# aleju/face-generator

Hardware: AMD Instinct MI355X
Metric: GAN train images/sec (G+D step) at 32x32x3 bs128 (higher is better)
Workload: dtype f32

## Files before the change

### face_generator_amd/csrc/igemm.hip

```cpp
#include "fg_internal.h"
#include <stdio.h>
#include <stdlib.h>

typedef float f32x16 __attribute__((ext_vector_type(16)));

__device__ __forceinline__ void fg_decode_m(int m, int lgH, int lgW, int Hm, int Wm, int& n, int& y, int& x) {
    if (lgW >= 0) {
        x = m & (Wm - 1);
        y = (m >> lgW) & (Hm - 1);
        n = m >> (lgW + lgH);
    } else {
        x = m % Wm;
        int t = m / Wm;
        y = t % Hm;
        n = t / Hm;
    }
}

typedef unsigned int u32x4 __attribute__((ext_vector_type(4)));
#define FG_OOB 0x7FFFFFF0
#define FG_ROW_MASKED 0x20000000

typedef float f32x2 __attribute__((ext_vector_type(2)));
typedef float f32x4 __attribute__((ext_vector_type(4)));
// ... 1720 lines not shown
        }
        for (; s < S; ++s) sum += b[(size_t)s * tile];
    };
    if (wm.kind == 0) {
        run(Part + (size_t)wi * S * tile + e);
    } else {
        for (int p = 0; p < 4; ++p) {
            const int ty = dev_fold_r(p >> 1, dy, wm.pad) - wm.rmin;
            const int tx = dev_fold_r(p & 1, dx, wm.pad) - wm.rmin;
            const int pg = p * wm.G + ty * wm.T + tx;
            run(Part + (size_t)pg * S * tile + e);
        }
    }
    float* gw = gradW + ((size_t)o * wm.I + i) * wm.k * wm.k + wi;
    *gw = (beta == 0.f) ? sum : beta * (*gw) + sum;
}
__host__ __device__ static inline bool fg_finish_all_taps(const WeightMap& wm) { return !wm.wino && wm.kind == 0 && (wm.k == 3 || wm.k == 5); }
__host__ __device__ static inline int fg_finish_taps_tpb(int S) { return S >= 12 ? 32 : 128; }
template <int K>
__device__ __forceinline__ void wgrad_finish_taps(const WeightMap& wm, const float* __restrict__ Part, int S, int Npad, int Cpad,
                                                  float beta, float* __restrict__ gradW, int bx, int po, float* sh) {
    constexpr int kk = K * K;
    const int tpb = fg_finish_taps_tpb(S), ngrp = 128 / tpb;
    const int il = (int)threadIdx.x % tpb, q = (int)threadIdx.x / tpb;
    const int pi = bx * tpb + il;
    const size_t tile = (size_t)Npad * Cpad;
    const int per = (S + ngrp - 1) / ngrp, s0 = q * per, s1 = min(S, s0 + per);
    float sum[kk];
#pragma unroll
    for (int wi = 0; wi < kk; ++wi) sum[wi] = 0.f;
    if (pi < wm.I && po < wm.O) {
        const float* __restrict__ b = Part + (size_t)po * Cpad + pi;
        int s = s0;
        for (; s + 2 <= s1; s += 2) {
            float v0[kk], v1[kk];
#pragma unroll
            for (int wi = 0; wi < kk; ++wi) {
                v0[wi] = b[((size_t)wi * S + s) * tile];
                v1[wi] = b[((size_t)wi * S + s + 1) * tile];
            }
#pragma unroll
            for (int wi = 0; wi < kk; ++wi) { sum[wi] += v0[wi]; sum[wi] += v1[wi]; }
        }
        if (s < s1) {
#pragma unroll
            for (int wi = 0; wi < kk; ++wi) sum[wi] += b[((size_t)wi * S + s) * tile];
        }
    }
#pragma unroll
    for (int wi = 0; wi < kk; ++wi) sh[(q * tpb + il) * kk + wi] = sum[wi];
    __syncthreads();
    if (po >= wm.O) return;
    const int nI = min(tpb, wm.I - bx * tpb);
    float* __restrict__ base = gradW + ((size_t)po * wm.I + (size_t)bx * tpb) * kk;
    for (int idx = (int)threadIdx.x; idx < nI * kk; idx += 128) {
        float t = sh[idx];
        for (int g = 1; g < ngrp; ++g) t += sh[g * tpb * kk + idx];
        base[idx] = (beta == 0.f) ? t : beta * base[idx] + t;
    }
}
__device__ __forceinline__ void wgrad_finish_taps_any(const WeightMap& wm, const float* __restrict__ Part, int S, int Npad, int Cpad,
                                                      float beta, float* __restrict__ gradW, int bx, int po, float* sh) {
    if (wm.k == 5) wgrad_finish_taps<5>(wm, Part, S, Npad, Cpad, beta, gradW, bx, po, sh);
    else wgrad_finish_taps<3>(wm, Part, S, Npad, Cpad, beta, gradW, bx, po, sh);
}
#define FG_WINO_FINISH_LDS (25 * 128)
__host__ __device__ static inline int fg_wino_finish_tpu(const WeightMap& wm) { return (wm.kind == 1 || wm.wino == 2) ? 32 : 128; }
template <int K>
__device__ __forceinline__ void wino_wgrad_finish_block(const WeightMap& wm, const float* __restrict__ Part, int S, int Npad, int Cpad,
                                                        float beta, float* __restrict__ gradW, int bx, int o, float* sh) {
    const int units = (wm.kind == 1 ? 4 : 1) * (wm.wino == 2 ? 4 : 1);
    const int tpu = fg_wino_finish_tpu(wm);
    const int tid = threadIdx.x, u = units == 1 ? 0 : tid / tpu, il = units == 1 ? tid : tid - u * tpu;
    const int i = bx * tpu + il;
    const bool live = i < wm.I && o < wm.O;
    const size_t tile = (size_t)Npad * Cpad;
    float g[K * K];
#pragma unroll
    for (int q = 0; q < K * K; ++q) g[q] = 0.f;
    if (live) {
        float du[16];
#pragma unroll
        for (int pos = 0; pos < 16; ++pos) du[pos] = 0.f;
        const float4* __restrict__ b = (const float4*)(Part + ((size_t)u * S * tile + (size_t)o * Cpad + i) * 16);
        int s = 0;
        for (; s + 4 <= S; s += 4) {
            float4 v[4][4];
#pragma unroll
            for (int e = 0; e < 4; ++e)
#pragma unroll
                for (int q = 0; q < 4; ++q) v[e][q] = b[(size_t)(s + e) * tile * 4 + q];
#pragma unroll
            for (int e = 0; e < 4; ++e)
#pragma unroll
                for (int q = 0; q < 4; ++q) { du[4 * q] += v[e][q].x; du[4 * q + 1] += v[e][q].y; du[4 * q + 2] += v[e][q].z; du[4 * q + 3] += v[e][q].w; }
        }
        for (; s < S; ++s) {
            float4 v[4];
#pragma unroll
            for (int q = 0; q < 4; ++q) v[q] = b[(size_t)s * tile * 4 + q];
#pragma unroll
            for (int q = 0; q < 4; ++q) { du[4 * q] += v[q].x; du[4 * q + 1] += v[q].y; du[4 * q + 2] += v[q].z; du[4 * q + 3] += v[q].w; }
        }
#pragma unroll
        for (int pos = 0; pos < 16; ++pos)
            if (((pos >> 2) == 3) != ((pos & 3) == 3)) du[pos] = -du[pos];
        float r[4][3], t[9];
#pragma unroll
        for (int ii = 0; ii < 4; ++ii) {
            const float d0 = du[ii * 4], d1 = du[ii * 4 + 1], d2 = du[ii * 4 + 2], d3 = du[ii * 4 + 3];
            r[ii][0] = d0 + 0.5f * (d1 + d2);
            r[ii][1] = 0.5f * (d1 - d2);
            r[ii][2] = 0.5f * (d1 + d2) + d3;
        }
#pragma unroll
        for (int bb = 0; bb < 3; ++bb) {
            t[0 * 3 + bb] = r[0][bb] + 0.5f * (r[1][bb] + r[2][bb]);
            t[1 * 3 + bb] = 0.5f * (r[1][bb] - r[2][bb]);
            t[2 * 3 + bb] = 0.5f * (r[1][bb] + r[2][bb]) + r[3][bb];
        }
        if (K == 5 && wm.wino == 2) {
#pragma unroll
            for (int dy = 0; dy < 3; ++dy)
#pragma unroll
                for (int dx = 0; dx < 3; ++dx)
#pragma unroll
                    for (int q = 0; q < K * K; ++q)
                        g[q] = (q == (3 * (u >> 1) + dy) * K + 3 * (u & 1) + dx && 3 * (u >> 1) + dy < K && 3 * (u & 1) + dx < K) ? t[dy * 3 + dx] : g[q];
        } else if (wm.kind == 1) {
#pragma unroll
            for (int dy = 0; dy < K; ++dy)
#pragma unroll
                for (int dx = 0; dx < K; ++dx) {
                    const int ty = dev_fold_r(u >> 1, dy, wm.pad) - wm.rmin, tx = dev_fold_r(u & 1, dx, wm.pad) - wm.rmin;
                    float v = 0.f;
#pragma unroll
                    for (int q = 0; q < 9; ++q) v = (ty * 3 + tx == q) ? t[q] : v;
                    g[dy * K + dx] = v;
                }
        } else if (K == 3) {
#pragma unroll
            for (int q = 0; q < 9; ++q) g[q] = t[q];
        }
    }
    if (units > 1) {
#pragma unroll
        for (int q = 0; q < K * K; ++q) sh[q * 128 + tid] = g[q];
        __syncthreads();
        if (u != 0 || !live) return;
#pragma unroll
        for (int q = 0; q < K * K; ++q) g[q] = ((sh[q * 128 + il] + sh[q * 128 + tpu + il]) + sh[q * 128 + 2 * tpu + il]) + sh[q * 128 + 3 * tpu + il];
    } else if (!live) return;
    float* gw = gradW + ((size_t)o * wm.I + i) * (K * K);
#pragma unroll
    for (int q = 0; q < K * K; ++q) gw[q] = (beta == 0.f) ? g[q] : beta * gw[q] + g[q];
}
__device__ __forceinline__ void wino_wgrad_finish_any(const WeightMap& wm, const float* __restrict__ Part, int S, int Npad, int Cpad,
                                                      float beta, float* __restrict__ gradW, int bx, int o, float* sh) {
    if (wm.k == 5) wino_wgrad_finish_block<5>(wm, Part, S, Npad, Cpad, beta, gradW, bx, o, sh);
    else wino_wgrad_finish_block<3>(wm, Part, S, Npad, Cpad, beta, gradW, bx, o, sh);
}
struct FgWFinishBatch { FgWFinishJob jobs[FG_DEFER_WMAX]; int n; };
__global__ __launch_bounds__(128) void wgrad_finish_jobs_kernel(const FgWFinishBatch b) {
    __shared__ float tl[32][33];
    __shared__ float wsh[FG_WINO_FINISH_LDS];
    int j = 0;
    while (j + 1 < b.n && (long long)blockIdx.x >= b.jobs[j + 1].blk0) ++j;
    const FgWFinishJob& jb = b.jobs[j];
    long long l = (long long)blockIdx.x - jb.blk0;
    if (jb.ib < 0) {
        const WeightMap& wm = jb.wm;
        const int C = wm.i_c, HW = wm.i_hw, nct = (C + 31) / 32, nht = (HW + 31) / 32;
        const int ht = (int)(l % nht); l /= nht;
        const int ct = (int)(l % nct);
        const int po = (int)(l / nct);
        int o = po;
        if (wm.o_hw > 1) { int hw = po / wm.o_c, c = po - hw * wm.o_c; o = c * wm.o_hw + hw; }
        const size_t tile = (size_t)jb.Npad * jb.Cpad;
        const int lx = threadIdx.x & 31, ly = threadIdx.x >> 5;
        for (int r = ly; r < 32; r += 4) {
            const int hw = ht * 32 + r, c = ct * 32 + lx;
            float sum = 0.f;
            if (hw < HW && c < C) {
// ... 489 lines not shown
```

### face_generator_amd/csrc/wino.hip

```cpp
#include "fg_internal.h"
#include <stdio.h>
#include <stdlib.h>
#include <vector>

typedef float f32x16 __attribute__((ext_vector_type(16)));
typedef float f32x4 __attribute__((ext_vector_type(4)));
typedef float f32x2 __attribute__((ext_vector_type(2)));
#define FG_OOB 0x7FFFFFF0

#define WN_STAGE 16384

__device__ __forceinline__ f32x2 wn_load2(__amdgpu_buffer_rsrc_t r, int voff, int soff) {
    return __builtin_bit_cast(f32x2, __builtin_amdgcn_raw_buffer_load_b64(r, voff, soff, 0));
}
__device__ __forceinline__ f32x4 wn_load4(__amdgpu_buffer_rsrc_t r, int voff, int soff) {
    return __builtin_bit_cast(f32x4, __builtin_amdgcn_raw_buffer_load_b128(r, voff, soff, 0));
}
__device__ __forceinline__ f32x2 wn_add(f32x2 a, f32x2 b) {
    f32x2 d;
    asm("v_pk_add_f32 %0, %1, %2" : "=v"(d) : "v"(a), "v"(b));
    return d;
}
__device__ __forceinline__ f32x2 wn_sub(f32x2 a, f32x2 b) {
    f32x2 d;
    asm("v_pk_add_f32 %0, %1, %2 neg_lo:[0,1] neg_hi:[0,1]" : "=v"(d) : "v"(a), "v"(b));
    return d;
}
__device__ __forceinline__ void wn_decode(int t, const WinoArgs& a, int& b, int& ty, int& tx) {
    if (a.lgTW >= 0) {
        tx = t & (a.TW - 1);
        ty = (t >> a.lgTW) & (a.TH - 1);
        b = t >> (a.lgTW + a.lgTH);
    } else {
        tx = t % a.TW;
        const int q = t / a.TW;
        ty = q % a.TH;
        b = q / a.TH;
    }
}

template <int EPI, int TRACE = 0, int DBG = 0>
__device__ __forceinline__ void wino_body(const WinoArgs& a) {
    extern __shared__ __attribute__((aligned(16))) float smem[];
    int* rowoff = (int*)(smem + 2 * WN_STAGE);

    const int tid = threadIdx.x, lane = tid & 63;
    const int wid = __builtin_amdgcn_readfirstlane(tid >> 6);
    const int wm = wid >> 1, wn = wid & 1;
    const int nbn = a.Npad >> 6;
    const int ntn = nbn * a.P;
    const int nmt = (a.T + 63) >> 6;
    int lin = blockIdx.x;
    if ((nmt & 7) == 0) {
        const int xcd = lin & 7, loc = lin >> 3;
        lin = (xcd * (nmt >> 3) + loc / ntn) * ntn + loc % ntn;
    }
    const int tile_m = lin / ntn, cb = lin - tile_m * ntn;
    const int par = cb / nbn, tile_n = cb - par * nbn;
    const int nch = a.C >> 3;
    const int nct = nch * a.KG;
    const int per = (nct + a.splits - 1) / a.splits;
    const int c0 = blockIdx.y * per;
    const int NC = max(0, min(nct, c0 + per) - c0);

    if (tid < 64) {
        const int t = tile_m * 64 + tid;
        int off = -1;
        if (t < a.T) {
            int b, ty, tx;
            wn_decode(t, a, b, ty, tx);
            off = ((b * a.Ho + a.osy * 2 * ty + a.ooy[par]) * a.Wo + a.osx * 2 * tx + a.oox[par]) * a.N;
        }
        rowoff[tid] = off;
    }

    const __amdgpu_buffer_rsrc_t xrsrc = __builtin_amdgcn_make_buffer_rsrc((void*)a.X, 0, (int)a.x_bytes, 0x00020000);
    const __amdgpu_buffer_rsrc_t ursrc = __builtin_amdgcn_make_buffer_rsrc((void*)a.U, 0, FG_OOB, 0x00020000);
    const __amdgpu_buffer_rsrc_t zrsrc = __builtin_amdgcn_make_buffer_rsrc((void*)a.U, 0, 0, 0x00020000);
    const int NCE = (NC + 1) & ~1;
    int voff[16];
    int pb, py0, px0;
    bool tvalid;
    {
        const int t = tile_m * 64 + (tid >> 2);
        int b, ty, tx;
        tvalid = t < a.T;
        wn_decode(tvalid ? t : 0, a, b, ty, tx);
        pb = b * a.Hi; py0 = a.isy * 2 * ty; px0 = a.isx * 2 * tx;
    }
    const int goy4 = *(const int*)a.goy, gox4 = *(const int*)a.gox;
#define WN_GOFF(pk, g) ((int)(signed char)((pk) >> (8 * (g))))
    const int cstep = a.isx * a.C * 4;
#define WN_SET_GROUP(g)                                                                                    \
    {                                                                                                      \
        const int gy_ = py0 + WN_GOFF(goy4, g), gx_ = px0 + WN_GOFF(gox4, g);                              \
        int rb_[4]; bool rok_[4], cok_[4];                                                                 \
        _Pragma("unroll") for (int i = 0; i < 4; ++i) {                                                    \
            const int y = gy_ + a.isy * i;                                                                 \
            rok_[i] = tvalid & ((unsigned)y < (unsigned)a.Hi);                                              \
            rb_[i] = (((pb + y) * a.Wi + gx_) * a.C + 2 * (tid & 3)) * 4;                                  \
            cok_[i] = (unsigned)(gx_ + a.isx * i) < (unsigned)a.Wi;                                        \
        }                                                                                                  \
        _Pragma("unroll") for (int p = 0; p < 16; ++p) voff[p] = (rok_[p >> 2] & cok_[p & 3]) ? rb_[p >> 2] + (p & 3) * cstep : FG_OOB; \
    }
    const int vw = ((tid & 3) >> 1) * 256 + (tid >> 2) * 4 + (tid & 1) * 2;
    const int uo = tid * 4;
    const int ubase = (par * nbn + tile_n) * nct;
    const int a_rd = (lane >> 5) * 256 + (wm * 32 + (lane & 31)) * 4;
    const int b_rd = 8192 + (lane >> 5) * 256 + (wn * 32 + (lane & 31)) * 4;

    int cl = c0, gl = c0 / nch, ccl = c0 - gl * nch;
    WN_SET_GROUP(gl < a.KG ? gl : 0);
#define WN_ADVANCE()                                                                                       \
    {                                                                                                      \
        ++cl;                                                                                              \
        if (++ccl == nch) { ccl = 0; ++gl; if (gl < a.KG) WN_SET_GROUP(gl); }                              \
    }

    f32x2 rva[16], rvb[16];
    f32x4 rua[8], rub[8];
#define WN_LOAD(rv, ru)                                                                                    \
    {                                                                                                      \
        const int sx = ccl * 32, su = (ubase + cl) * 32768;                                                \
        const bool real_ = cl < c0 + NC;                                                                   \
        const __amdgpu_buffer_rsrc_t xr_ = real_ ? xrsrc : zrsrc, ur_ = real_ ? ursrc : zrsrc;             \
        _Pragma("unroll") for (int p = 0; p < 16; ++p) rv[p] = wn_load2(xr_, voff[p], sx);                 \
        _Pragma("unroll") for (int i = 0; i < 8; ++i) ru[i] = wn_load4(ur_, (uo + i * 1024) * 4, su);       \
    }
#define WN_XFORM_STORE(S, rv, ru)                                                                          \
    {                                                                                                      \
        float* Vs = (S) + vw;                                                                              \
        float* Us = (S) + 8192 + uo;                                                                       \
        _Pragma("unroll") for (int i = 0; i < 8; ++i) *(f32x4*)(Us + i * 1024) = ru[i];                    \
        f32x2 w_[16];                                                                                      \
        _Pragma("unroll") for (int x = 0; x < 4; ++x) {                                                    \
            w_[0 + x] = rv[0 + x] - rv[8 + x];                                                             \
            w_[4 + x] = rv[4 + x] + rv[8 + x];                                                             \
            w_[8 + x] = rv[8 + x] - rv[4 + x];                                                             \
            w_[12 + x] = rv[4 + x] - rv[12 + x];                                                           \
        }                                                                                                  \
        _Pragma("unroll") for (int i = 0; i < 4; ++i) {                                                    \
            *(f32x2*)(Vs + (i * 4 + 0) * 512) = w_[i * 4 + 0] - w_[i * 4 + 2];                             \
            *(f32x2*)(Vs + (i * 4 + 1) * 512) = w_[i * 4 + 1] + w_[i * 4 + 2];                             \
            *(f32x2*)(Vs + (i * 4 + 2) * 512) = w_[i * 4 + 2] - w_[i * 4 + 1];                             \
            *(f32x2*)(Vs + (i * 4 + 3) * 512) = w_[i * 4 + 1] - w_[i * 4 + 3];                             \
        }                                                                                                  \
    }

    const int col = tile_n * 64 + wn * 32 + (lane & 31);
    const bool colok = col < a.N;
    const bool bias_late = a.stats_part != nullptr;
    const float bv = (a.bias != nullptr && a.splits == 1 && colok) ? a.bias[col] : 0.f;
    f32x16 acc[16];
#pragma unroll
    for (int p = 0; p < 16; ++p)
#pragma unroll
        for (int r = 0; r < 16; ++r) acc[p][r] = (p == 5 && !bias_late) ? bv : 0.f;

    f32x4 fa[2][2], fb[2][2];
    unsigned long long* trc = nullptr;
    if (TRACE) {
        if (wid == 0 && a.dbg_trace) trc = a.dbg_trace + (size_t)(blockIdx.x + gridDim.x * blockIdx.y) * 128;
        if (trc && lane == 0) trc[0] = __builtin_amdgcn_s_memtime();
    }
    if (NC > 0) {
        WN_LOAD(rva, rua); WN_ADVANCE();
        WN_LOAD(rvb, rub); WN_ADVANCE();
    }
#pragma unroll
    for (int p = 0; p < 16; ++p) asm volatile("" : "+a"(acc[p]));
    __builtin_amdgcn_sched_barrier(0);
    if (NC > 0) {
        WN_XFORM_STORE(smem, rva, rua);
    }
    asm volatile("s_waitcnt lgkmcnt(0)\n\ts_barrier" ::: "memory");
    if (TRACE && trc && lane == 0) trc[1] = __builtin_amdgcn_s_memtime();
    if (NC > 0) {
#pragma unroll
        for (int h = 0; h < 2; ++h) {
            fa[0][h] = *(const f32x4*)(smem + a_rd + h * 512);
            fb[0][h] = *(const f32x4*)(smem + b_rd + h * 512);
        }
    }

#define WN_CHUNK(HAS1, HAS2, RX, UX, RY, UY)                                                               \
    {                                                                                                      \
        const float* Sc = smem + s * WN_STAGE;                                                             \
        float* Sn = smem + (s ^ 1) * WN_STAGE;                                                             \
        float* Vs = Sn + vw;                                                                               \
        float* Us = Sn + 8192 + uo;                                                                        \
        const int sx2 = ccl * 32, su2 = (ubase + cl) * 32768;                                              \
        const bool real_ = cl < c0 + NC;                                                                   \
        const __amdgpu_buffer_rsrc_t xr_ = real_ ? xrsrc : zrsrc, ur_ = real_ ? ursrc : zrsrc;             \
        f32x2 t_;                                                                                          \
        _Pragma("unroll") for (int pr = 0; pr < 8; ++pr) {                                                 \
            _Pragma("unroll") for (int m = 0; m < 8; ++m) {                                                \
                const int sl = pr * 8 + m, h = m & 1, j = m >> 1, pos = 2 * pr + h;                        \
                acc[pos] = __builtin_amdgcn_mfma_f32_32x32x2f32(fa[pr & 1][h][j], fb[pr & 1][h][j], acc[pos], 0, 0, 0); \
                if (TRACE == 2 && (sl & 7) == 0 && ci < 14) {                                              \
                    if (trc && lane == 0) trc[8 + ci * 8 + (sl >> 3)] = __builtin_amdgcn_s_memtime();       \
                }                                                                                          \
                if (m < 4 && pr < 7 && !(DBG & 8)) {                                                       \
                    const int np = 2 * (pr + 1) + (m >> 1);                                                \
                    if ((m & 1) == 0) fa[(pr + 1) & 1][m >> 1] = *(const f32x4*)(Sc + a_rd + np * 512);    \
                    else fb[(pr + 1) & 1][m >> 1] = *(const f32x4*)(Sc + b_rd + np * 512);                 \
                }                                                                                          \
                if (HAS1) {                                                                                \
                    if (m < 4 && pr == 7 && !(DBG & 8)) {                                                  \
                        if ((m & 1) == 0) fa[0][m >> 1] = *(const f32x4*)(Sn + a_rd + (m >> 1) * 512);     \
                        else fb[0][m >> 1] = *(const f32x4*)(Sn + b_rd + (m >> 1) * 512);                  \
                    }                                                                                      \
                    if (sl < 8 && !(DBG & 1)) *(f32x4*)(Us + sl * 1024) = UX[sl];                          \
                    if (HAS2 && !(DBG & 4)) {             \
                        if (sl < 16 && (sl & 1) == 0) UY[sl >> 1] = wn_load4(ur_, (uo + (sl >> 1) * 1024) * 4, su2); \
                        if (sl >= 9 && sl < 41 && (sl & 1) == 1) RY[(sl - 9) >> 1] = wn_load2(xr_, voff[(sl - 9) >> 1], sx2); \
                    }                                                                                      \
                                \
                    if (sl == 8 && !(DBG & 2)) {                                                           \
                        _Pragma("unroll") for (int x = 0; x < 4; ++x) {                                    \
                            RX[0 + x] = wn_sub(RX[0 + x], RX[8 + x]);                                      \
                            RX[12 + x] = wn_sub(RX[4 + x], RX[12 + x]);                                    \
                            t_ = wn_add(RX[4 + x], RX[8 + x]);                                             \
                            RX[8 + x] = wn_sub(RX[8 + x], RX[4 + x]); RX[4 + x] = t_;                      \
                        }                                                                                  \
                    }                                                                                      \
                    if (sl == 10 && !(DBG & 2)) {                                                          \
                        _Pragma("unroll") for (int i = 0; i < 4; ++i) {                                    \
                            RX[i * 4 + 0] = wn_sub(RX[i * 4 + 0], RX[i * 4 + 2]);                          \
                            RX[i * 4 + 3] = wn_sub(RX[i * 4 + 1], RX[i * 4 + 3]);                          \
                            t_ = wn_add(RX[i * 4 + 1], RX[i * 4 + 2]);                                     \
                            RX[i * 4 + 2] = wn_sub(RX[i * 4 + 2], RX[i * 4 + 1]); RX[i * 4 + 1] = t_;      \
                        }                                                                                  \
                    }                                                                                      \
                    if (sl >= 12 && sl < 28 && !(DBG & 2)) *(f32x2*)(Vs + (sl - 12) * 512) = RX[sl - 12];  \
                    if (sl == 55) asm volatile("s_waitcnt lgkmcnt(0)\n\ts_barrier" ::: "memory");          \
                }                                                                                          \
                __builtin_amdgcn_sched_barrier(0);                                                         \
            }                                                                                              \
        }                                                                                                  \
    }
#define WN_STAMP() { if (TRACE == 1 && trc && lane == 0) trc[2 + (ci < 119 ? ci : 119)] = __builtin_amdgcn_s_memtime(); ++ci; }
    int s = 0;
    int ci = 0;
    if (NCE > 0) {
        for (; ci + 2 < NCE;) {
            WN_CHUNK(true, true, rvb, rub, rva, rua); WN_ADVANCE(); WN_STAMP();
            s ^= 1;
            WN_CHUNK(true, true, rva, rua, rvb, rub); WN_ADVANCE(); WN_STAMP();
            s ^= 1;
        }
        WN_CHUNK(true, false, rvb, rub, rva, rua); WN_STAMP();
        s ^= 1;
        WN_CHUNK(false, false, rva, rua, rvb, rub);
        if (ci < NC) WN_STAMP();
    }
#undef WN_STAMP
#undef WN_SET_GROUP
#undef WN_GOFF
#undef WN_ADVANCE
#undef WN_LOAD
#undef WN_XFORM_STORE
#undef WN_CHUNK

    float* outp = a.Out + (size_t)blockIdx.y * a.split_stride;
    const __amdgpu_buffer_rsrc_t orsrc = __builtin_amdgcn_make_buffer_rsrc((void*)outp, 0, FG_OOB, 0x00020000);
    const int oN = a.osx * a.N * 4, oW = a.osy * a.Wo * a.N * 4;
    float sl_ = 0.f, ssum = 0.f, st1 = 0.f, st2 = 0.f;
    if (EPI != 0) sl_ = a.act_slope[0];
    const float badd = bias_late ? bv : 0.f;
#pragma unroll
    for (int r4 = 0; r4 < 4; ++r4) {
        const int4 ro4 = *(const int4*)(rowoff + wm * 32 + 8 * r4 + 4 * (lane >> 5));
        const int ros[4] = {ro4.x, ro4.y, ro4.z, ro4.w};
        float xv[4][4];
        if (EPI == 2) {
            const __amdgpu_buffer_rsrc_t xr = __builtin_amdgcn_make_buffer_rsrc((void*)a.act_x, 0, FG_OOB, 0x00020000);
#pragma unroll
            for (int q = 0; q < 4; ++q) {
                const int vo = (ros[q] >= 0 && colok) ? (ros[q] + col) * 4 : FG_OOB;
                xv[q][0] = __uint_as_float(__builtin_amdgcn_raw_buffer_load_b32(xr, vo, 0, 0));
                xv[q][1] = __uint_as_float(__builtin_amdgcn_raw_buffer_load_b32(xr, vo, oN, 0));
                xv[q][2] = __uint_as_float(__builtin_amdgcn_raw_buffer_load_b32(xr, vo, oW, 0));
                xv[q][3] = __uint_as_float(__builtin_amdgcn_raw_buffer_load_b32(xr, vo, oW + oN, 0));
            }
        }
#pragma unroll
        for (int q = 0; q < 4; ++q) {
            __builtin_amdgcn_sched_barrier(0);
            const int r = r4 * 4 + q;
            float t0[4], t1[4];
#pragma unroll
            for (int j = 0; j < 4; ++j) {
                t0[j] = (acc[0 + j][r] + acc[4 + j][r]) + acc[8 + j][r];
                t1[j] = (acc[4 + j][r] - acc[8 + j][r]) - acc[12 + j][r];
            }
            float y[4];
            y[0] = (t0[0] + t0[1]) + t0[2];
            y[1] = (t0[1] - t0[2]) - t0[3];
            y[2] = (t1[0] + t1[1]) + t1[2];
            y[3] = (t1[1] - t1[2]) - t1[3];
            const int vo = (ros[q] >= 0 && colok) ? (ros[q] + col) * 4 : FG_OOB;
            const int so[4] = {0, oN, oW, oW + oN};
#pragma unroll
            for (int e = 0; e < 4; ++e) {
                if (EPI == 2) {
                    const float x = xv[q][e];
                    const bool pos = x > 0.f;
                    ssum = fmaf(pos ? 0.f : x, y[e], ssum);
                    __builtin_amdgcn_raw_buffer_store_b32(__float_as_uint(pos ? y[e] : sl_ * y[e]), orsrc, vo, so[e], 0);
                } else {
                    if (bias_late) {
                        st1 += y[e];
                        st2 = fmaf(y[e], y[e], st2);
                    }
                    const float yo = y[e] + badd;
                    __builtin_amdgcn_raw_buffer_store_b32(__float_as_uint(yo), orsrc, vo, so[e], 0);
                    if (EPI == 1) {
                        const __amdgpu_buffer_rsrc_t yr = __builtin_amdgcn_make_buffer_rsrc((void*)a.act_y, 0, FG_OOB, 0x00020000);
                        __builtin_amdgcn_raw_buffer_store_b32(__float_as_uint(yo > 0.f ? yo : sl_ * yo), yr, vo, so[e], 0);
                    }
                }
            }
        }
    }
    if (EPI == 2 && a.act_part) {
#pragma unroll
        for (int o = 32; o > 0; o >>= 1) ssum += __shfl_xor(ssum, o, 64);
        if (lane == 0) a.act_part[blockIdx.x * 4 + wid] = ssum;
    }
    if (EPI != 2 && bias_late) {
        st1 += __shfl_xor(st1, 32, 64);
        st2 += __shfl_xor(st2, 32, 64);
        const int row = (tile_m * a.P + par) * 2 + wm;
        if (lane < 32 && colok) {
            a.stats_part[(size_t)row * a.N + col] = st1;
            a.stats_part[((size_t)a.stats_rows + row) * a.N + col] = st2;
        }
    }
    if (TRACE && trc && lane == 0) {
        __builtin_amdgcn_s_waitcnt(0x0f70);
        if (TRACE == 1) trc[(NC < 120 ? NC : 120) + 2] = __builtin_amdgcn_s_memtime();
        trc[127] = (unsigned long long)__builtin_amdgcn_s_getreg(((3 - 1) << 11) | (0 << 6) | 20) | ((unsigned long long)NC << 32);
        trc[126] = (unsigned long long)__builtin_amdgcn_s_getreg(((32 - 1) << 11) | (0 << 6) | 4);
// ... 112 lines not shown
```

### face_generator_amd/csrc/wino_wgrad.hip

```cpp
#include "fg_internal.h"
#include <stdio.h>
#include <stdlib.h>
#include <vector>

typedef float f32x16 __attribute__((ext_vector_type(16)));
typedef float f32x4 __attribute__((ext_vector_type(4)));
typedef float f32x2 __attribute__((ext_vector_type(2)));
#define FG_OOB 0x7FFFFFF0
#define WW_STAGE 16384

__device__ __forceinline__ float ww_load(__amdgpu_buffer_rsrc_t r, int voff, int soff) {
    return __uint_as_float(__builtin_amdgcn_raw_buffer_load_b32(r, voff, soff, 0));
}
__device__ __forceinline__ f32x2 ww_add(f32x2 a, f32x2 b) {
    f32x2 d;
    asm("v_pk_add_f32 %0, %1, %2" : "=v"(d) : "v"(a), "v"(b));
    return d;
}
__device__ __forceinline__ f32x2 ww_sub(f32x2 a, f32x2 b) {
    f32x2 d;
    asm("v_pk_add_f32 %0, %1, %2 neg_lo:[0,1] neg_hi:[0,1]" : "=v"(d) : "v"(a), "v"(b));
    return d;
}

template <int TRACE>
__device__ __forceinline__ void ww_body(const WinoWgradArgs& a) {
    extern __shared__ __attribute__((aligned(16))) float smem[];
    const int tid = threadIdx.x, lane = tid & 63;
    const int wid = __builtin_amdgcn_readfirstlane(tid >> 6);
    const int wm = wid >> 1, wn = wid & 1;
    const int nbc = a.Cpad >> 6;
    const int tn = blockIdx.x / nbc, tc = blockIdx.x - tn * nbc;
    const int pg = blockIdx.z, par = pg / a.KG, grp = pg - par * a.KG;
    const int nct = (a.T + 7) >> 3;
    const int c0 = blockIdx.y * a.chunks_per_split;
    const int NC = max(0, min(nct, c0 + a.chunks_per_split) - c0);
    const int NCE = (NC + 1) & ~1;
    if (NC <= 0) return;
    unsigned long long* trc = nullptr;
    if (TRACE) {
        if (wid == 0 && a.dbg_trace) trc = a.dbg_trace + ((size_t)blockIdx.x + (size_t)gridDim.x * (blockIdx.y + (size_t)gridDim.y * blockIdx.z)) * 128;
        if (trc && lane == 0) trc[0] = __builtin_amdgcn_s_memtime();
    }
    int ci = 0;

    const int dRow = a.osy * a.Wo * a.Nd * 4, dCol = a.osx * a.Nd * 4;
    const int xRow = a.isy * a.Wi * a.Cx * 4, xCol = a.isx * a.Cx * 4;
    const int xShift = 2 * a.Cx * 4;
    const __amdgpu_buffer_rsrc_t drsrc = __builtin_amdgcn_make_buffer_rsrc((void*)a.dY, 0, (int)a.d_bytes, 0x00020000);
    const __amdgpu_buffer_rsrc_t xrsrc = __builtin_amdgcn_make_buffer_rsrc((void*)((const char*)a.X - xShift), 0, (int)a.x_bytes + xShift, 0x00020000);
    const int chD = tn * 64 + lane, chX = tc * 64 + lane;
    const int vD = chD < a.Nd ? chD * 4 : FG_OOB, vX = chX < a.Cx ? chX * 4 : FG_OOB;
    const int goy = a.goy[grp], gox = a.gox[grp], ooy = a.ooy[par], oox = a.oox[par];
    const int cend = c0 + NC;

    const int sw = (wid >> 1) * 256 + lane * 4 + (wid & 1) * 2;
    const int a_rd = (lane >> 5) * 256 + (wm * 32 + (lane & 31)) * 4;
    const int b_rd = 8192 + (lane >> 5) * 256 + (wn * 32 + (lane & 31)) * 4;

    int cl = c0;
    int vrow[4], vdr[2], vo[24], colmask = 0;
    int cur_b = 0, cur_y0 = 0, cur_x0 = 0, cur_dy = 0, cur_dx = 0, cur_tv = 0;
#define WW_CURSOR_A()                                                                                      \
    {                                                                                                      \
        const int t0 = cl * 8 + 2 * wid;                              \
        cur_tv = (t0 < a.T && cl < cend) ? 1 : 0;                                                          \
        const int tt = cur_tv ? t0 : 0;                                                                    \
        const int tx = tt & (a.TW - 1), ty = (tt >> a.lgTW) & (a.TH - 1);                                  \
        cur_b = tt >> (a.lgTW + a.lgTH);                                                                   \
        cur_y0 = a.isy * 2 * ty + goy; cur_x0 = a.isx * 2 * tx + gox;                                      \
        cur_dy = a.osy * 2 * ty + ooy; cur_dx = a.osx * 2 * tx + oox;                                      \
    }
#define WW_CURSOR_B()                                                                                      \
    {                                                                                                      \
        const int rowbase = ((cur_b * a.Hi + cur_y0) * a.Wi + cur_x0) * a.Cx * 4 + xShift;                 \
        _Pragma("unroll") for (int i = 0; i < 4; ++i)                                                      \
            vrow[i] = (cur_tv && (unsigned)(cur_y0 + a.isy * i) < (unsigned)a.Hi) ? vX + (rowbase + i * xRow) : FG_OOB; \
        colmask = 0;                                                                                       \
        _Pragma("unroll") for (int j = 0; j < 6; ++j) if ((unsigned)(cur_x0 + a.isx * j) < (unsigned)a.Wi) colmask |= 1 << j; \
        const int dbase = ((cur_b * a.Ho + cur_dy) * a.Wo + cur_dx) * a.Nd * 4;                            \
        vdr[0] = cur_tv ? vD + dbase : FG_OOB;                                                             \
        vdr[1] = cur_tv ? vD + (dbase + dRow) : FG_OOB;                                                    \
    }
#define WW_CURSOR_C(I0)                                                                                    \
    {                                                                                                      \
        _Pragma("unroll") for (int i = (I0); i < (I0) + 2; ++i)                                            \
            _Pragma("unroll") for (int j = 0; j < 6; ++j) vo[i * 6 + j] = ((colmask >> j) & 1) ? vrow[i] : FG_OOB; \
    }
#define WW_CURSOR() { WW_CURSOR_A(); WW_CURSOR_B(); WW_CURSOR_C(0); WW_CURSOR_C(2); }
#define WW_LDX(i, j, h) ww_load(xrsrc, vo[(i) * 6 + (j) + 2 * (h)], ((j) + 2 * (h)) * xCol)
#define WW_LDD(r, e, h) ww_load(drsrc, vdr[r], ((e) + 2 * (h)) * dCol)

    f32x2 xa[16], xb[16], da[4], db[4];
#define WW_LOAD_ALL(xs, ds)                                                                                \
    {                                                                                                      \
        _Pragma("unroll") for (int q = 0; q < 4; ++q) { ds[q].x = WW_LDD(q >> 1, q & 1, 0); ds[q].y = WW_LDD(q >> 1, q & 1, 1); } \
        _Pragma("unroll") for (int q = 0; q < 16; ++q) { xs[q].x = WW_LDX(q >> 2, q & 3, 0); xs[q].y = WW_LDX(q >> 2, q & 3, 1); } \
    }
#define WW_XFORM_STORE(S, xs, ds)                                                                          \
    {                                                                                                      \
        float* Ms = (S) + sw;                                                                              \
        float* Vs = (S) + 8192 + sw;                                                                       \
        f32x2 u_[8];                                                                                       \
        _Pragma("unroll") for (int e = 0; e < 2; ++e) {                                                    \
            u_[0 + e] = ds[0 + e]; u_[2 + e] = ds[0 + e] + ds[2 + e]; u_[4 + e] = ds[0 + e] - ds[2 + e]; u_[6 + e] = ds[2 + e]; \
        }                                                                                                  \
        _Pragma("unroll") for (int i = 0; i < 4; ++i) {                                                    \
            *(f32x2*)(Ms + (i * 4 + 0) * 512) = u_[i * 2];                                                 \
            *(f32x2*)(Ms + (i * 4 + 1) * 512) = u_[i * 2] + u_[i * 2 + 1];                                 \
            *(f32x2*)(Ms + (i * 4 + 2) * 512) = u_[i * 2] - u_[i * 2 + 1];                                 \
            *(f32x2*)(Ms + (i * 4 + 3) * 512) = u_[i * 2 + 1];                                             \
        }                                                                                                  \
        f32x2 w_[16];                                                                                      \
        _Pragma("unroll") for (int x = 0; x < 4; ++x) {                                                    \
            w_[0 + x] = xs[0 + x] - xs[8 + x];                                                             \
            w_[4 + x] = xs[4 + x] + xs[8 + x];                                                             \
            w_[8 + x] = xs[8 + x] - xs[4 + x];                                                             \
            w_[12 + x] = xs[4 + x] - xs[12 + x];                                                           \
        }                                                                                                  \
        _Pragma("unroll") for (int i = 0; i < 4; ++i) {                                                    \
            *(f32x2*)(Vs + (i * 4 + 0) * 512) = w_[i * 4 + 0] - w_[i * 4 + 2];                             \
            *(f32x2*)(Vs + (i * 4 + 1) * 512) = w_[i * 4 + 1] + w_[i * 4 + 2];                             \
            *(f32x2*)(Vs + (i * 4 + 2) * 512) = w_[i * 4 + 2] - w_[i * 4 + 1];                             \
            *(f32x2*)(Vs + (i * 4 + 3) * 512) = w_[i * 4 + 1] - w_[i * 4 + 3];                             \
        }                                                                                                  \
    }

    f32x16 acc[16];
#pragma unroll
    for (int p = 0; p < 16; ++p)
#pragma unroll
        for (int r = 0; r < 16; ++r) acc[p][r] = 0.f;
    f32x2 bsum = {0.f, 0.f};

    f32x4 fa[2][2], fb[2][2];
    if (NC > 0) {
// ... 40 lines not shown
                }                                                                                          \
                if (HAS1) {                                                                                \
                    if (m < 4 && pr == 7) {                                                                \
                        if ((m & 1) == 0) fa[0][m >> 1] = *(const f32x4*)(Sn + a_rd + (m >> 1) * 512);     \
                        else fb[0][m >> 1] = *(const f32x4*)(Sn + b_rd + (m >> 1) * 512);                  \
                    }                                                                                      \
                    if (HAS2) {                                                                            \
                        if (sl >= 1 && sl < 5) {                                                           \
                            const int q = sl - 1;                                                          \
                            DL[q].x = WW_LDD(q >> 1, q & 1, 0); DL[q].y = WW_LDD(q >> 1, q & 1, 1);        \
                        }                                                                                  \
                        if (sl >= 5 && sl < 37) {                                                          \
                            const int q = (sl - 5) >> 1, hh = (sl - 5) & 1;                                \
                            if (hh == 0) XL[q].x = WW_LDX(q >> 2, q & 3, 0); else XL[q].y = WW_LDX(q >> 2, q & 3, 1); \
                        }                                                                                  \
                    }                                                                                      \
                    if (HAS2 && sl == 57) { ++cl; WW_CURSOR_A(); }      \
                    if (HAS2 && sl == 58) { WW_CURSOR_B(); }                                               \
                    if (HAS2 && sl == 60) { WW_CURSOR_C(0); }                                              \
                    if (HAS2 && sl == 61) { WW_CURSOR_C(2); }                                              \
                                         \
                    if (sl == 0) {                                                                         \
                        bsum = ww_add(bsum, ww_add(ww_add(DS[0], DS[1]), ww_add(DS[2], DS[3])));           \
                        u_[0] = DS[0]; u_[1] = DS[1]; u_[6] = DS[2]; u_[7] = DS[3];                        \
                        u_[2] = ww_add(DS[0], DS[2]); u_[3] = ww_add(DS[1], DS[3]);                        \
                        u_[4] = ww_sub(DS[0], DS[2]); u_[5] = ww_sub(DS[1], DS[3]);                        \
                        _Pragma("unroll") for (int i = 0; i < 4; ++i) {                                    \
                            m_[i * 4 + 0] = u_[i * 2]; m_[i * 4 + 3] = u_[i * 2 + 1];                      \
                            m_[i * 4 + 1] = ww_add(u_[i * 2], u_[i * 2 + 1]);                              \
                            m_[i * 4 + 2] = ww_sub(u_[i * 2], u_[i * 2 + 1]);                              \
                        }                                                                                  \
                    }                                                                                      \
                    if (sl >= 2 && sl < 18) *(f32x2*)(Ms + (sl - 2) * 512) = m_[sl - 2];                   \
                          \
                    if (sl == 19) {                                                                        \
                        _Pragma("unroll") for (int x = 0; x < 4; ++x) {                                    \
                            XS[0 + x] = ww_sub(XS[0 + x], XS[8 + x]);                                      \
                            XS[12 + x] = ww_sub(XS[4 + x], XS[12 + x]);                                    \
                            t_ = ww_add(XS[4 + x], XS[8 + x]);                                             \
                            XS[8 + x] = ww_sub(XS[8 + x], XS[4 + x]); XS[4 + x] = t_;                      \
                        }                                                                                  \
                    }                                                                                      \
                    if (sl == 21) {                                                                        \
                        _Pragma("unroll") for (int i = 0; i < 4; ++i) {                                    \
                            XS[i * 4 + 0] = ww_sub(XS[i * 4 + 0], XS[i * 4 + 2]);                          \
                            XS[i * 4 + 3] = ww_sub(XS[i * 4 + 1], XS[i * 4 + 3]);                          \
                            t_ = ww_add(XS[i * 4 + 1], XS[i * 4 + 2]);                                     \
                            XS[i * 4 + 2] = ww_sub(XS[i * 4 + 2], XS[i * 4 + 1]); XS[i * 4 + 1] = t_;      \
                        }                                                                                  \
                    }                                                                                      \
                    if (sl >= 23 && sl < 39) *(f32x2*)(Vs + (sl - 23) * 512) = XS[sl - 23];                \
                    if (sl == 55) asm volatile("s_waitcnt lgkmcnt(0)\n\ts_barrier" ::: "memory");          \
                }                                                                                          \
                __builtin_amdgcn_sched_barrier(0);                                                         \
            }                                                                                              \
        }                                                                                                  \
    }
    int s = 0;
    if (NCE > 0) {
        for (; ci + 2 < NCE;) {
            WW_CHUNK(true, true, xb, db, xa, da);
            WW_STAMP();
            s ^= 1;
            WW_CHUNK(true, true, xa, da, xb, db);
            WW_STAMP();
            s ^= 1;
        }
        WW_CHUNK(true, false, xb, db, xa, da);
        WW_STAMP();
        s ^= 1;
        WW_CHUNK(false, false, xa, da, xb, db);
        WW_STAMP();
    }
#undef WW_CURSOR
#undef WW_CURSOR_A
#undef WW_CURSOR_B
#undef WW_LDX
#undef WW_LDD
#undef WW_LOAD_ALL
#undef WW_XFORM_STORE
#undef WW_CHUNK

    {
        float* outp = a.Part + (((size_t)pg * a.S + blockIdx.y) * 16) * (size_t)a.Npad * a.Cpad;
        const __amdgpu_buffer_rsrc_t orsrc = __builtin_amdgcn_make_buffer_rsrc((void*)outp, 0, FG_OOB, 0x00020000);
        const int col = tc * 64 + wn * 32 + (lane & 31);
        const int row0 = tn * 64 + wm * 32 + 4 * (lane >> 5);
#pragma unroll
        for (int r = 0; r < 16; ++r) {
            const int row = row0 + (r & 3) + 8 * (r >> 2);
            const int vo = (row * a.Cpad + col) * 64;
            __builtin_amdgcn_sched_barrier(0);
#pragma unroll
            for (int q = 0; q < 4; ++q) {
                const f32x4 v = {acc[4 * q][r], acc[4 * q + 1][r], acc[4 * q + 2][r], acc[4 * q + 3][r]};
                __builtin_amdgcn_raw_buffer_store_b128(__builtin_bit_cast(__attribute__((__vector_size__(4 * sizeof(unsigned)))) unsigned, v), orsrc, vo, q * 16, 0);
            }
        }
    }
    if (a.bias_part && tc == 0 && grp == 0) {
        __syncthreads();
        float* red = smem;
        red[wid * 64 + lane] = bsum.x + bsum.y;
        __syncthreads();
        if (wid == 0 && chD < a.Nd)
            a.bias_part[((size_t)par * a.S + blockIdx.y) * a.Nd + chD] = (red[lane] + red[64 + lane]) + (red[128 + lane] + red[192 + lane]);
    }
    if (TRACE && trc && lane == 0) {
        asm volatile("s_waitcnt vmcnt(0)" ::: "memory");
        if (TRACE == 1) trc[(NC < 120 ? NC : 120) + 2] = __builtin_amdgcn_s_memtime();
        trc[127] = (unsigned long long)__builtin_amdgcn_s_getreg(((3 - 1) << 11) | (0 << 6) | 20) | ((unsigned long long)NC << 32);
        trc[126] = (unsigned long long)__builtin_amdgcn_s_getreg(((32 - 1) << 11) | (0 << 6) | 4);
    }
#undef WW_STAMP
}
__global__ __launch_bounds__(256) void wino_wgrad_kernel(const WinoWgradArgs a) { ww_body<0>(a); }
#ifdef FG_MEASURE
template <int TRACE>
__global__ __launch_bounds__(256) void wino_wgrad_trace_kernel(const WinoWgradArgs a) { ww_body<TRACE>(a); }

static int ww_trace_launch(fg_ctx* ctx, const WinoWgradArgs& a_in, dim3 grid, size_t lds, int mode) {
    WinoWgradArgs a = a_in;
    const size_t nblk = (size_t)grid.x * grid.y * grid.z;
    unsigned long long* dvc = nullptr;
    if (hipMalloc((void**)&dvc, nblk * 128 * 8) != hipSuccess) return fg_set_err(ctx, FG_ERR_NOMEM, "trace buffer");
    (void)hipMemset(dvc, 0, nblk * 128 * 8);
    a.dbg_trace = dvc;
    hipEvent_t e0, e1;
    (void)hipEventCreate(&e0); (void)hipEventCreate(&e1);
    (void)hipFuncSetAttribute((const void*)wino_wgrad_trace_kernel<1>, hipFuncAttributeMaxDynamicSharedMemorySize, (int)lds);
    (void)hipFuncSetAttribute((const void*)wino_wgrad_trace_kernel<2>, hipFuncAttributeMaxDynamicSharedMemorySize, (int)lds);
    for (int rep = 0; rep < 4; ++rep) {
        (void)hipEventRecord(e0, ctx->stream);
        if (mode == 2) hipLaunchKernelGGL(wino_wgrad_trace_kernel<2>, grid, dim3(256), lds, ctx->stream, a);
        else hipLaunchKernelGGL(wino_wgrad_trace_kernel<1>, grid, dim3(256), lds, ctx->stream, a);
        (void)hipEventRecord(e1, ctx->stream);
    }
    FG_CHECK_LAUNCH(ctx);
    FG_HIP(ctx, hipStreamSynchronize(ctx->stream));
    float wall_ms = 0.f;
    (void)hipEventElapsedTime(&wall_ms, e0, e1);
    (void)hipEventDestroy(e0); (void)hipEventDestroy(e1);
    std::vector<unsigned long long> host(nblk * 128);
    FG_HIP(ctx, hipMemcpy(host.data(), dvc, nblk * 128 * 8, hipMemcpyDeviceToHost));
    (void)hipFree(dvc);
    const char* path = getenv("FG_WS_TRACE_FILE");
    FILE* f = fopen(path ? path : "/tmp/fg_ws_trace.txt", "a");
    if (f) {
        fprintf(f, "# launch wino_wgrad(dbg=%d)/%s BN=128 blocks=%zu T=%d Npad=%d Cpad=%d units=%d S=%d wall_us=%.1f\n", mode == 2 ? 100 : 0, a.tag ? a.tag : "?", nblk,
                a.T, a.Npad, a.Cpad, a.P * a.KG, a.S, wall_ms * 1e3);
        for (size_t b = 0; b < nblk; ++b) {
            const unsigned long long* r = host.data() + b * 128;
            const int kt = (int)(r[127] >> 32), xcc = (int)(r[127] & 0xffffffff);
            fprintf(f, "%zu %d %d %llu", b, xcc, kt, r[126]);
            if (mode == 2) { for (int i = 0; i < 126; ++i) fprintf(f, " %llu", r[i]); }
            else for (int i = 0; i < (kt < 120 ? kt : 120) + 3; ++i) fprintf(f, " %llu", r[i]);
            fprintf(f, "\n");
        }
        fclose(f);
    }
    return FG_OK;
}
#endif

int fg_launch_wino_wgrad(fg_ctx* ctx, const WinoWgradArgs& a) {
    if (a.chunks_per_split < 1 || (long long)(a.S - 1) * a.chunks_per_split >= (a.T + 7) / 8)
        return fg_set_err(ctx, FG_ERR_INVALID, "winograd wgrad: a split without chunks (S = %d x %d chunks, %d tiles)", a.S, a.chunks_per_split, a.T);
    if (a.Npad % 64 || a.Cpad % 64 || a.S < 1 || a.lgTW < 1 || a.lgTH < 0 || a.P < 1 || a.KG < 1 || a.P * a.KG > 4)
        return fg_set_err(ctx, FG_ERR_INVALID, "winograd wgrad: padded channels %% 64, power-of-two tile grid (>= 2 wide), <= 4 units");
    if (a.x_bytes <= 0 || a.x_bytes + 8LL * a.Cx >= (long long)FG_OOB || a.d_bytes <= 0 || a.d_bytes >= (long long)FG_OOB)
        return fg_set_err(ctx, FG_ERR_UNSUPPORTED, "winograd wgrad: operands must be < 2 GiB per launch");
    const size_t lds = (size_t)(2 * WW_STAGE) * sizeof(float);
    static char attr_key;
    if (fg_attr_first(ctx, &attr_key)) {
        FG_HIP(ctx, hipFuncSetAttribute((const void*)wino_wgrad_kernel, hipFuncAttributeMaxDynamicSharedMemorySize, (int)lds));
    }
    dim3 grid((a.Npad / 64) * (a.Cpad / 64), a.S, a.P * a.KG);
    const double exec = 2.0 * (double)a.Nd * a.Cx * grid.z * 16.0 * (double)a.T;
#ifdef FG_MEASURE
// ... 14 lines not shown
```

Measured before the change: 49400.

## Use plane-major Winograd wgrad partial layout and prefetch U before setup

The Winograd weight-gradient partial buffer changes from a per-element 16-float interleaved layout to four separate planes, one per float4 quad, each of size tile. Writer stores and finisher loads become contiguous across lanes, with each quad offset by q*tile. In the forward Winograd kernel, the first U-tile loads are issued before address setup and the rowoff computation is moved after the initial loads to hide latency. Small per-parity/group offsets are now read as packed bytes, which removes indexed scalar loads. The risk is the larger scalar offset (q*tile*16) used in the buffer stores.

```diff
diff --git a/face_generator_amd/csrc/igemm.hip b/face_generator_amd/csrc/igemm.hip
--- a/face_generator_amd/csrc/igemm.hip
+++ b/face_generator_amd/csrc/igemm.hip
@@ -1826,14 +1826,14 @@
         float du[16];
 #pragma unroll
         for (int pos = 0; pos < 16; ++pos) du[pos] = 0.f;
-        const float4* __restrict__ b = (const float4*)(Part + ((size_t)u * S * tile + (size_t)o * Cpad + i) * 16);
+        const float4* __restrict__ b = (const float4*)Part + (size_t)u * S * tile * 4 + (size_t)o * Cpad + i;
         int s = 0;
         for (; s + 4 <= S; s += 4) {
             float4 v[4][4];
 #pragma unroll
             for (int e = 0; e < 4; ++e)
 #pragma unroll
-                for (int q = 0; q < 4; ++q) v[e][q] = b[(size_t)(s + e) * tile * 4 + q];
+                for (int q = 0; q < 4; ++q) v[e][q] = b[((size_t)(s + e) * 4 + q) * tile];
 #pragma unroll
             for (int e = 0; e < 4; ++e)
 #pragma unroll
@@ -1842,7 +1842,7 @@
         for (; s < S; ++s) {
             float4 v[4];
 #pragma unroll
-            for (int q = 0; q < 4; ++q) v[q] = b[(size_t)s * tile * 4 + q];
+            for (int q = 0; q < 4; ++q) v[q] = b[((size_t)s * 4 + q) * tile];
 #pragma unroll
             for (int q = 0; q < 4; ++q) { du[4 * q] += v[q].x; du[4 * q + 1] += v[q].y; du[4 * q + 2] += v[q].z; du[4 * q + 3] += v[q].w; }
         }
diff --git a/face_generator_amd/csrc/wino.hip b/face_generator_amd/csrc/wino.hip
--- a/face_generator_amd/csrc/wino.hip
+++ b/face_generator_amd/csrc/wino.hip
@@ -62,22 +62,28 @@
     const int per = (nct + a.splits - 1) / a.splits;
     const int c0 = blockIdx.y * per;
     const int NC = max(0, min(nct, c0 + per) - c0);
-
-    if (tid < 64) {
-        const int t = tile_m * 64 + tid;
-        int off = -1;
-        if (t < a.T) {
-            int b, ty, tx;
-            wn_decode(t, a, b, ty, tx);
-            off = ((b * a.Ho + a.osy * 2 * ty + a.ooy[par]) * a.Wo + a.osx * 2 * tx + a.oox[par]) * a.N;
-        }
-        rowoff[tid] = off;
+    unsigned long long* trc = nullptr;
+    if (TRACE) {
+        if (wid == 0 && a.dbg_trace) trc = a.dbg_trace + (size_t)(blockIdx.x + gridDim.x * blockIdx.y) * 128;
+        if (trc && lane == 0) trc[0] = __builtin_amdgcn_s_memtime();
     }
 
     const __amdgpu_buffer_rsrc_t xrsrc = __builtin_amdgcn_make_buffer_rsrc((void*)a.X, 0, (int)a.x_bytes, 0x00020000);
     const __amdgpu_buffer_rsrc_t ursrc = __builtin_amdgcn_make_buffer_rsrc((void*)a.U, 0, FG_OOB, 0x00020000);
     const __amdgpu_buffer_rsrc_t zrsrc = __builtin_amdgcn_make_buffer_rsrc((void*)a.U, 0, 0, 0x00020000);
     const int NCE = (NC + 1) & ~1;
+    const int uo = tid * 4;
+    const int ubase = (par * nbn + tile_n) * nct;
+    f32x2 rva[16], rvb[16];
+    f32x4 rua[8], rub[8];
+#define WN_LOAD_U(ru, c)                                                                                   \
+    {                                                                                                      \
+        const int su = (ubase + (c)) * 32768;                                                              \
+        const __amdgpu_buffer_rsrc_t ur_ = (c) < c0 + NC ? ursrc : zrsrc;                                  \
+        _Pragma("unroll") for (int i = 0; i < 8; ++i) ru[i] = wn_load4(ur_, (uo + i * 1024) * 4, su);       \
+    }
+    if (NC > 0) WN_LOAD_U(rua, c0);
+    __builtin_amdgcn_sched_barrier(0);
     int voff[16];
     int pb, py0, px0;
     bool tvalid;
@@ -104,8 +110,6 @@
         _Pragma("unroll") for (int p = 0; p < 16; ++p) voff[p] = (rok_[p >> 2] & cok_[p & 3]) ? rb_[p >> 2] + (p & 3) * cstep : FG_OOB; \
     }
     const int vw = ((tid & 3) >> 1) * 256 + (tid >> 2) * 4 + (tid & 1) * 2;
-    const int uo = tid * 4;
-    const int ubase = (par * nbn + tile_n) * nct;
     const int a_rd = (lane >> 5) * 256 + (wm * 32 + (lane & 31)) * 4;
     const int b_rd = 8192 + (lane >> 5) * 256 + (wn * 32 + (lane & 31)) * 4;
 
@@ -117,15 +121,11 @@
         if (++ccl == nch) { ccl = 0; ++gl; if (gl < a.KG) WN_SET_GROUP(gl); }                              \
     }
 
-    f32x2 rva[16], rvb[16];
-    f32x4 rua[8], rub[8];
-#define WN_LOAD(rv, ru)                                                                                    \
-    {                                                                                                      \
-        const int sx = ccl * 32, su = (ubase + cl) * 32768;                                                \
-        const bool real_ = cl < c0 + NC;                                                                   \
-        const __amdgpu_buffer_rsrc_t xr_ = real_ ? xrsrc : zrsrc, ur_ = real_ ? ursrc : zrsrc;             \
+#define WN_LOAD_X(rv)                                                                                      \
+    {                                                                                                      \
+        const int sx = ccl * 32;                                                                           \
+        const __amdgpu_buffer_rsrc_t xr_ = cl < c0 + NC ? xrsrc : zrsrc;                                   \
         _Pragma("unroll") for (int p = 0; p < 16; ++p) rv[p] = wn_load2(xr_, voff[p], sx);                 \
-        _Pragma("unroll") for (int i = 0; i < 8; ++i) ru[i] = wn_load4(ur_, (uo + i * 1024) * 4, su);       \
     }
 #define WN_XFORM_STORE(S, rv, ru)                                                                          \
     {                                                                                                      \
@@ -158,14 +158,20 @@
         for (int r = 0; r < 16; ++r) acc[p][r] = (p == 5 && !bias_late) ? bv : 0.f;
 
     f32x4 fa[2][2], fb[2][2];
-    unsigned long long* trc = nullptr;
-    if (TRACE) {
-        if (wid == 0 && a.dbg_trace) trc = a.dbg_trace + (size_t)(blockIdx.x + gridDim.x * blockIdx.y) * 128;
-        if (trc && lane == 0) trc[0] = __builtin_amdgcn_s_memtime();
-    }
     if (NC > 0) {
-        WN_LOAD(rva, rua); WN_ADVANCE();
-        WN_LOAD(rvb, rub); WN_ADVANCE();
+        WN_LOAD_X(rva); WN_ADVANCE();
+        WN_LOAD_U(rub, cl); WN_LOAD_X(rvb); WN_ADVANCE();
+    }
+    if (tid < 64) {
+        const int t = tile_m * 64 + tid;
+        int off = -1;
+        if (t < a.T) {
+            int b, ty, tx;
+            wn_decode(t, a, b, ty, tx);
+            const int ooy4 = *(const int*)a.ooy, oox4 = *(const int*)a.oox;
+            off = ((b * a.Ho + a.osy * 2 * ty + WN_GOFF(ooy4, par)) * a.Wo + a.osx * 2 * tx + WN_GOFF(oox4, par)) * a.N;
+        }
+        rowoff[tid] = off;
     }
 #pragma unroll
     for (int p = 0; p < 16; ++p) asm volatile("" : "+a"(acc[p]));
@@ -258,7 +264,8 @@
 #undef WN_SET_GROUP
 #undef WN_GOFF
 #undef WN_ADVANCE
-#undef WN_LOAD
+#undef WN_LOAD_U
+#undef WN_LOAD_X
 #undef WN_XFORM_STORE
 #undef WN_CHUNK
 
diff --git a/face_generator_amd/csrc/wino_wgrad.hip b/face_generator_amd/csrc/wino_wgrad.hip
--- a/face_generator_amd/csrc/wino_wgrad.hip
+++ b/face_generator_amd/csrc/wino_wgrad.hip
@@ -51,7 +51,10 @@
     const __amdgpu_buffer_rsrc_t xrsrc = __builtin_amdgcn_make_buffer_rsrc((void*)((const char*)a.X - xShift), 0, (int)a.x_bytes + xShift, 0x00020000);
     const int chD = tn * 64 + lane, chX = tc * 64 + lane;
     const int vD = chD < a.Nd ? chD * 4 : FG_OOB, vX = chX < a.Cx ? chX * 4 : FG_OOB;
-    const int goy = a.goy[grp], gox = a.gox[grp], ooy = a.ooy[par], oox = a.oox[par];
+#define WW_BYTE(pk, g) ((int)(signed char)((pk) >> (8 * (g))))
+    const int goy = WW_BYTE(*(const int*)a.goy, grp), gox = WW_BYTE(*(const int*)a.gox, grp);
+    const int ooy = WW_BYTE(*(const int*)a.ooy, par), oox = WW_BYTE(*(const int*)a.oox, par);
+#undef WW_BYTE
     const int cend = c0 + NC;
 
     const int sw = (wid >> 1) * 256 + lane * 4 + (wid & 1) * 2;
@@ -258,19 +261,20 @@
 #undef WW_CHUNK
 
     {
-        float* outp = a.Part + (((size_t)pg * a.S + blockIdx.y) * 16) * (size_t)a.Npad * a.Cpad;
+        const int tile = a.Npad * a.Cpad;
+        float* outp = a.Part + (((size_t)pg * a.S + blockIdx.y) * 16) * (size_t)tile;
         const __amdgpu_buffer_rsrc_t orsrc = __builtin_amdgcn_make_buffer_rsrc((void*)outp, 0, FG_OOB, 0x00020000);
         const int col = tc * 64 + wn * 32 + (lane & 31);
         const int row0 = tn * 64 + wm * 32 + 4 * (lane >> 5);
 #pragma unroll
         for (int r = 0; r < 16; ++r) {
             const int row = row0 + (r & 3) + 8 * (r >> 2);
-            const int vo = (row * a.Cpad + col) * 64;
+            const int vo = (row * a.Cpad + col) * 16;
             __builtin_amdgcn_sched_barrier(0);
 #pragma unroll
             for (int q = 0; q < 4; ++q) {
                 const f32x4 v = {acc[4 * q][r], acc[4 * q + 1][r], acc[4 * q + 2][r], acc[4 * q + 3][r]};
-                __builtin_amdgcn_raw_buffer_store_b128(__builtin_bit_cast(__attribute__((__vector_size__(4 * sizeof(unsigned)))) unsigned, v), orsrc, vo, q * 16, 0);
+                __builtin_amdgcn_raw_buffer_store_b128(__builtin_bit_cast(__attribute__((__vector_size__(4 * sizeof(unsigned)))) unsigned, v), orsrc, vo, q * tile * 16, 0);
             }
         }
     }
```

After: 50210, median of 6. 1.02x the previous value.
